# Tamnemng/TAM-GCN

Hardware: AMD Instinct MI355X
Metric: skeleton clips/sec (fwd+CE+bwd+grad all-reduce+SGD step), N-UCLA 20-joint x 64-frame (higher is better)
Workload: dtype f32 (exact fp32-input MFMA v_mfma_f32_16x16x4_f32 in every GEMM, forward and backward: the reference's arithmetic); 1 GPU; N-UCLA joint stream, 256 clips/GPU x (3,64,20,1), models.ctrgcn.Model fwd+CE+bwd+grad-allreduce+SGD step, train-mode BN; global_batch=256, streams=1, parallelism=dp1, launch=hipgraph, model_streams=0, rehearsal=False, allreduce=one flat bucket after backward

## Files before the change

### tam_gcn_amd/csrc/conv.hip

```cpp
#include "common.h"

namespace {

constexpr int BM = 64;
constexpr int BK = 16;
constexpr int BKP = BK + 1;
constexpr int MAXCW = 5;
constexpr int MAXCOLS = 320;

TG_TRACE_DEFINE(tamgcn_trace_read)

struct ConvArgs {
    SrcDev src;
    int N, K, T_in, V;
    const float* w; const float* bias;
    int M, KT, dil, stride, pad;
    long long ws_m, ws_k, ws_t, w_off;
    int up, wmode;
    float* y; int yctot, ycoff, T_out, T_y, ostride;
    const float* add1; const float* add2; const float* bcast; float bcast_scale;
    SrcDev mask; int has_mask;
    const float* aux; const float* aux_center; int auxctot, auxcoff;
    float* stats_part; int stats_ctot, stats_coff, nparts;
    const float* post_coef; int post_ctot, post_act;
// ... 118 lines not shown
    const int V = a.V;
    const int bt = min(a.BT, a.T_out - t0);
    const int ncols = bt * V;
    const int nct = (ncols + 15) >> 4;
    const int cw0 = wave * a.CW;
    const int mt_act = min(4, (min(BM, a.M - m0) + 15) >> 4);
    int c_act = nct - cw0; c_act = c_act < 0 ? 0 : (c_act > a.CW ? a.CW : c_act);

    int boff[MAXCW], tl[MAXCW], vv[MAXCW];
#pragma unroll
    for (int c = 0; c < MAXCW; ++c) {
        int col = (cw0 + c) * 16 + j;
        if (col < ncols) { tl[c] = col / V; vv[c] = col - tl[c] * V; boff[c] = tl[c] * a.sB * V + vv[c]; }
        else { tl[c] = 0; vv[c] = 0; boff[c] = 0; }
    }

    f32x4 acc[4][MAXCW];
#pragma unroll
    for (int mt = 0; mt < 4; ++mt)
#pragma unroll
        for (int c = 0; c < MAXCW; ++c) acc[mt][c] = (f32x4){0.f, 0.f, 0.f, 0.f};

    const int tin0 = t0 * a.stride - a.pad;
    const long long chan_stride = (long long)a.T_in * V;
    const long long src_n = (long long)n * a.src.ctot * chan_stride;

    for (int k0 = 0; k0 < a.K; k0 += BK) {
        __syncthreads();
        const int nA = a.KT * BM * BK;
        for (int e = tid; e < nA; e += NTHREADS) {
            int kk = e & (BK - 1);
            int i = (e >> 4) & (BM - 1);
            int tap = e >> 10;
            int m = m0 + i, k = k0 + kk;
            float wv = 0.f;
            if (m < a.M && k < a.K) wv = a.w[m * a.ws_m + k * a.ws_k + tap * a.ws_t + a.w_off];
            As[(tap * BM + i) * BKP + kk] = wv;
        }
        for (int pos = tid; pos < a.LB; pos += NTHREADS) {
            int slot = pos / V;
            int v = pos - slot * V;
            int th = tin0 + slot * a.lstride;
            bool ok = th >= 0;
            if (a.up > 1) { ok = ok && (th % a.up == 0); th /= a.up; }
            ok = ok && th < a.T_in;
            long long goff = src_n + (long long)th * V + v;
#pragma unroll 4
            for (int kk = 0; kk < BK; ++kk) {
                int k = k0 + kk;
                float xv = 0.f;
                if (ok && k < a.K) {
                    int ch = a.src.coff + k;
                    xv = src_value(a.src, goff + ch * chan_stride, ch);
                }
                Bs[kk * a.pitchB + pos] = xv;
            }
        }
        __syncthreads();
        for (int tap = 0; tap < a.KT; ++tap) {
            const int tapoff = tap * a.dil * V;
#pragma unroll
            for (int k4 = 0; k4 < BK / 4; ++k4) {
                float av[4];
#pragma unroll
                for (int mt = 0; mt < 4; ++mt)
                    av[mt] = As[(tap * BM + mt * 16 + j) * BKP + k4 * 4 + kq];
                const float* brow = Bs + (k4 * 4 + kq) * a.pitchB + tapoff;
#pragma unroll
                for (int c = 0; c < MAXCW; ++c) {
                    if (c < c_act) {
                        float bv = brow[boff[c]];
#pragma unroll
                        for (int mt = 0; mt < 4; ++mt)
                            if (mt < mt_act) acc[mt][c] = mfma16(av[mt], bv, acc[mt][c]);
                    }
                }
            }
        }
    }

    conv_epilogue(a, acc, Ss, n, m0, t0, ncols, cw0, mt_act, c_act, tl, vv, j, kq, wave, tid);
}

template <int NTH, int PR = 0, typename SIDE = PairArgs>
__device__ __forceinline__ void staged_rows(const ConvArgs& a, const float* Tt, int PT, int RP, int r0, int BMT, int m0, int n, int t0,
                                            int ncols, float* Ss, int Vs, int v0, const SIDE* pa = nullptr) {
    const int tid = threadIdx.x, V = a.V;
    const int TPR = NTH / RP;
    const int row = tid / TPR, seg = tid - row * TPR;
    const int m = m0 + r0 + row;
    const bool flat = Vs == V && a.ostride == 1;
    const bool vecok = flat || (Vs & 3) == 0;
    float p1 = 0.f, p2 = 0.f;
    const bool rowok = r0 + row < BMT && m < a.M;
    if (rowok) {
        float bia = a.bias ? a.bias[m] : 0.f;
        float* yp = a.y;
        const float ctr = a.aux ? a.aux_center[a.auxcoff + m] : 0.f;
        const float pc1 = a.post_coef ? a.post_coef[a.ycoff + m] : 1.f, pc0 = a.post_coef ? a.post_coef[2 * a.post_ctot + a.ycoff + m] : 0.f;
        const float plo = a.post_act == 1 ? 0.f : -__builtin_inff();
        long long ybase = ((long long)n * a.yctot + a.ycoff + m) * a.T_y * V;
        if constexpr (PR == 1) {
            if (m >= pa->M0) {
                const int m1 = m - pa->M0;
                bia = pa->bias1 ? pa->bias1[m1] : 0.f; yp = pa->y1;
                ybase = ((long long)n * pa->yctot1 + pa->ycoff1 + m1) * a.T_y * V;
            }
        }
        const long long mbase = a.has_mask ? ((long long)n * a.mask.ctot + a.mask.coff + m) * a.T_y * V : 0;
        const unsigned char* sb = nullptr;
        if constexpr (PR == 2) sb = pa->bits + ((long long)n * pa->ctot + pa->coff + m) * ((a.T_y * V + 3) >> 2);
        const long long abase = a.aux ? ((long long)n * a.auxctot + a.auxcoff + m) * a.T_y * V : 0;
        const float* bc = a.bcast ? a.bcast + ((long long)m * a.N + n) * V : nullptr;
        float mc1 = 1.f, mc2 = 0.f, mc0 = 0.f;
        if (a.has_mask && a.mask.coef) {
            int mch = a.mask.coff + m;
            mc1 = a.mask.coef[mch]; mc0 = a.mask.coef[2 * a.mask.ctot + mch];
            if (a.mask.x2) mc2 = a.mask.coef[a.mask.ctot + mch];
        }
        const int nc4 = (ncols + 3) >> 2;
        unsigned snib = 0;
        if constexpr (PR == 2) {
            const unsigned char* sp = sb + ((t0 * V) >> 2);
#pragma unroll
            for (int k = 0; k < 6; ++k) {
                const int c = seg + k * TPR;
                snib |= (unsigned)sp[c < nc4 ? c : nc4 - 1] << (4 * k);
            }
        }
        int it = 0;
        for (int c4 = seg; c4 < nc4; c4 += TPR, ++it) {
            const int col = c4 << 2;
            const int fr = col / Vs, v = col - fr * Vs;
            if ((vecok || v + 4 <= Vs) && col + 4 <= ncols) {
                const long long off = (long long)(t0 + fr) * a.ostride * V + v0 + v;
                float4 val = *reinterpret_cast<const float4*>(Tt + row * PT + col);
                val.x = fmaf(pc1, val.x + bia, pc0); val.y = fmaf(pc1, val.y + bia, pc0);
                val.z = fmaf(pc1, val.z + bia, pc0); val.w = fmaf(pc1, val.w + bia, pc0);
                if (bc) {
                    float4 b;
                    if ((V & 3) == 0) b = *reinterpret_cast<const float4*>(bc + v0 + v);
                    else { const int j0 = (v0 + v) % V; b = make_float4(bc[j0], bc[(j0 + 1) % V], bc[(j0 + 2) % V], bc[(j0 + 3) % V]); }
                    val.x = fmaf(b.x, a.bcast_scale, val.x); val.y = fmaf(b.y, a.bcast_scale, val.y);
                    val.z = fmaf(b.z, a.bcast_scale, val.z); val.w = fmaf(b.w, a.bcast_scale, val.w);
                }
                if (a.add1) { float4 t = *reinterpret_cast<const float4*>(a.add1 + ybase + off); val.x += t.x; val.y += t.y; val.z += t.z; val.w += t.w; }
                if (a.add2) { float4 t = *reinterpret_cast<const float4*>(a.add2 + ybase + off); val.x += t.x; val.y += t.y; val.z += t.z; val.w += t.w; }
                val.x = fmaxf(val.x, plo); val.y = fmaxf(val.y, plo); val.z = fmaxf(val.z, plo); val.w = fmaxf(val.w, plo);
                if (a.has_mask) {
                    float4 q = *reinterpret_cast<const float4*>(a.mask.x1 + mbase + off);
                    float4 q2 = make_float4(0.f, 0.f, 0.f, 0.f);
                    if (a.mask.x2) q2 = *reinterpret_cast<const float4*>(a.mask.x2 + mbase + off);
                    if (!(fmaf(mc1, q.x, fmaf(mc2, q2.x, mc0)) > 0.f)) val.x = 0.f;
                    if (!(fmaf(mc1, q.y, fmaf(mc2, q2.y, mc0)) > 0.f)) val.y = 0.f;
                    if (!(fmaf(mc1, q.z, fmaf(mc2, q2.z, mc0)) > 0.f)) val.z = 0.f;
                    if (!(fmaf(mc1, q.w, fmaf(mc2, q2.w, mc0)) > 0.f)) val.w = 0.f;
                }
                if constexpr (PR == 2) {
                    const unsigned q = it < 6 ? snib >> (4 * it) : sb[off >> 2];
                    if (!(q & 1u)) val.x = 0.f;
                    if (!(q & 2u)) val.y = 0.f;
                    if (!(q & 4u)) val.z = 0.f;
                    if (!(q & 8u)) val.w = 0.f;
                }
                if (a.stats_part) {
                    float4 x2 = val;
                    if (a.aux) {
                        x2 = *reinterpret_cast<const float4*>(a.aux + abase + off);
                        x2.x -= ctr; x2.y -= ctr; x2.z -= ctr; x2.w -= ctr;
                    }
                    p1 += (val.x + val.y) + (val.z + val.w);
                    p2 = fmaf(val.x, x2.x, fmaf(val.y, x2.y, fmaf(val.z, x2.z, fmaf(val.w, x2.w, p2))));
                }
                *reinterpret_cast<float4*>(yp + ybase + off) = val;
            } else {
                for (int i = 0; i < 4 && col + i < ncols; ++i) {
                    const int ci = col + i, fi = ci / Vs, vi = ci - fi * Vs;
                    const long long off = (long long)(t0 + fi) * a.ostride * V + v0 + vi;
                    float val = fmaf(pc1, Tt[row * PT + ci] + bia, pc0);
                    if (bc) val = fmaf(bc[(v0 + vi) % V], a.bcast_scale, val);
                    if (a.add1) val += a.add1[ybase + off];
                    if (a.add2) val += a.add2[ybase + off];
                    val = fmaxf(val, plo);
                    if (a.has_mask) {
                        const float q = a.mask.x1[mbase + off], q2 = a.mask.x2 ? a.mask.x2[mbase + off] : 0.f;
                        if (!(fmaf(mc1, q, fmaf(mc2, q2, mc0)) > 0.f)) val = 0.f;
                    }
                    if constexpr (PR == 2) {
                        if (!((sb[off >> 2] >> (off & 3)) & 1u)) val = 0.f;
                    }
                    if (a.stats_part) {
                        const float x2 = a.aux ? a.aux[abase + off] - ctr : val;
                        p1 += val;
                        p2 = fmaf(val, x2, p2);
                    }
                    yp[ybase + off] = val;
                }
            }
        }
    }
    if (a.stats_part) {
        for (int o = 1; o < TPR; o <<= 1) { p1 += __shfl_xor(p1, o); p2 += __shfl_xor(p2, o); }
        if (seg == 0 && rowok) { Ss[r0 + row] = p1; Ss[4 * BM + r0 + row] = p2; }
    }
}

template <int BKV, int MT, int CWT>
__global__ __launch_bounds__(NTHREADS) void conv_kernel_vec(const ConvArgs a) {
    extern __shared__ __attribute__((aligned(16))) float smem[];
    constexpr int BKVP = BKV + 2;
    constexpr int BMT = MT * 16;
    constexpr int NPF = (BKV == 32) ? 10 : 8;
    float* As = smem;
    float* Bs = As + ((a.KT * BMT * BKVP + 3) & ~3);
    float* Ss = Bs + BKV * a.pitchB;
    float* cf = Ss + 2 * 4 * BM;

    const int tid = threadIdx.x, lane = tid & 63, wave = tid >> 6;
    const int j = lane & 15, kq = lane >> 4;
    const int tti = blockIdx.x / a.nsl, sl = blockIdx.x - tti * a.nsl;
    const int n = blockIdx.z, m0 = blockIdx.y * BMT, t0 = tti * a.BT;
    const int V = a.V, Vs = a.Vs, Vp = a.Vp, v0 = sl * Vs;
    const int bt = min(a.BT, a.T_out - t0);
    const int ncols = bt * Vs;
    const int cw0 = wave * CWT;

    for (int e = tid; e < a.K; e += NTHREADS) {
        int ch = a.src.coff + e;
        cf[e] = a.src.coef ? a.src.coef[ch] : 1.f;
        cf[a.K + e] = (a.src.coef && a.src.x2) ? a.src.coef[a.src.ctot + ch] : 0.f;
        cf[2 * a.K + e] = a.src.coef ? a.src.coef[2 * a.src.ctot + ch] : 0.f;
    }

    int boff[CWT], tl[CWT], vv[CWT];
#pragma unroll
    for (int c = 0; c < CWT; ++c) {
        int col = (cw0 + c) * 16 + j;
        if (col < ncols) { tl[c] = col / Vs; vv[c] = col - tl[c] * Vs; boff[c] = tl[c] * a.sB * Vp + vv[c]; }
        else { tl[c] = 0; vv[c] = 0; boff[c] = 0; }
    }
    f32x4 acc[MT][CWT];
#pragma unroll
    for (int mt = 0; mt < MT; ++mt)
#pragma unroll
        for (int c = 0; c < CWT; ++c) acc[mt][c] = (f32x4){0.f, 0.f, 0.f, 0.f};

    const int tin0 = t0 * a.stride - a.pad;
    const long long chan_stride = (long long)a.T_in * V;
    const int LB4 = a.LB >> 2;
    const int nvec = BKV * LB4;
    int p_lds[NPF], p_kk[NPF];
    long long p_g[NPF];
    bool p_ok[NPF];
#pragma unroll
    for (int i = 0; i < NPF; ++i) {
        int e = tid + i * NTHREADS;
        int kk = e / LB4, c4 = e - kk * LB4;
        int pos = c4 << 2;
        int slot = pos / Vp, v = pos - slot * Vp;
        int th = tin0 + slot * a.lstride;
        bool ok = e < nvec && th >= 0;
        if (a.up > 1) { ok = ok && (th % a.up == 0); th /= a.up; }
        ok = ok && th < a.T_in;
        p_ok[i] = ok;
        p_kk[i] = e < nvec ? kk : -1;
        p_lds[i] = kk * a.pitchB + pos;
        p_g[i] = (long long)n * a.src.ctot * chan_stride + (long long)(a.src.coff + kk) * chan_stride + (long long)th * V + v0 + v;
    }
    float4 r1[NPF], r2[NPF];
    const bool has2 = a.src.x2 != nullptr;
    constexpr int KTP = BKV == 16 ? 5 : 1;
    constexpr int NAF = (KTP * BMT * BKV + NTHREADS - 1) / NTHREADS;
    const bool apf = a.KT <= KTP;
    float wr[NAF];
    auto prefetch = [&](int k0) {
#pragma unroll
        for (int i = 0; i < NPF; ++i) {
            r1[i] = make_float4(0.f, 0.f, 0.f, 0.f);
            r2[i] = make_float4(0.f, 0.f, 0.f, 0.f);
            if (p_ok[i] && k0 + p_kk[i] < a.K) {
                long long g = p_g[i] + (long long)k0 * chan_stride;
                r1[i] = *reinterpret_cast<const float4*>(a.src.x1 + g);
                if (has2) r2[i] = *reinterpret_cast<const float4*>(a.src.x2 + g);
            }
        }
        if (apf) {
#pragma unroll
            for (int i = 0; i < NAF; ++i) {
// ... 23 lines not shown
        TG_T(tw); TG_ACC(2, tw - tb);
        const int nA = a.KT * BMT * BKV;
        if (apf) {
#pragma unroll
            for (int i = 0; i < NAF; ++i) {
                int e = tid + i * NTHREADS;
                const int tap = e / (BMT * BKV);
                e -= tap * (BMT * BKV);
                int ii, kk;
                if (a.wmode == 0) { kk = e % BKV; ii = e / BKV; } else { ii = e % BMT; kk = e / BMT; }
                if (tap < a.KT) As[(tap * BMT + ii) * BKVP + kk] = wr[i];
            }
        } else if (a.wmode == 0) {
            for (int e = tid; e < nA; e += NTHREADS) {
                int kk = e % BKV;
                int i = (e / BKV) % BMT;
                int tap = e / (BKV * BMT);
                int m = m0 + i, k = k0 + kk;
                float wv = 0.f;
                if (m < a.M && k < a.K) wv = a.w[m * a.ws_m + k * a.ws_k + tap * a.ws_t + a.w_off];
                As[(tap * BMT + i) * BKVP + kk] = wv;
            }
        } else {
            for (int e = tid; e < nA; e += NTHREADS) {
                int i = e % BMT;
                int kk = (e / BMT) % BKV;
                int tap = e / (BKV * BMT);
                int m = m0 + i, k = k0 + kk;
                float wv = 0.f;
                if (m < a.M && k < a.K) wv = a.w[m * a.ws_m + k * a.ws_k + tap * a.ws_t + a.w_off];
                As[(tap * BMT + i) * BKVP + kk] = wv;
            }
        }
#pragma unroll
        for (int i = 0; i < NPF; ++i) {
            if (p_kk[i] >= 0) {
                int k = k0 + p_kk[i];
                float4 o = make_float4(0.f, 0.f, 0.f, 0.f);
                if (p_ok[i] && k < a.K) {
                    float c1 = cf[k], c2 = cf[a.K + k], c0 = cf[2 * a.K + k];
                    o.x = fmaf(c1, r1[i].x, fmaf(c2, r2[i].x, c0)); o.y = fmaf(c1, r1[i].y, fmaf(c2, r2[i].y, c0));
                    o.z = fmaf(c1, r1[i].z, fmaf(c2, r2[i].z, c0)); o.w = fmaf(c1, r1[i].w, fmaf(c2, r2[i].w, c0));
                    if (a.src.act == 1) { o.x = fmaxf(o.x, 0.f); o.y = fmaxf(o.y, 0.f); o.z = fmaxf(o.z, 0.f); o.w = fmaxf(o.w, 0.f); }
                }
                *reinterpret_cast<float4*>(Bs + p_lds[i]) = o;
            }
        }
        TG_T(tc); TG_ACC(3, tc - tw);
        __syncthreads();
        TG_T(td); TG_ACC(4, td - tc);
        if (k0 + BKV < a.K) prefetch(k0 + BKV);
        TG_T(te); TG_ACC(5, te - td);
        for (int tap = 0; tap < a.KT; ++tap) {
            const float* at = arow + tap * BMT * BKVP;
            const float* bt_ = Bs + kq * a.pitchB + tap * a.dil * Vp;
#pragma unroll
            for (int k4 = 0; k4 < BKV / 4; ++k4) {
                float av[MT], bv[CWT];
#pragma unroll
                for (int mt = 0; mt < MT; ++mt) av[mt] = at[mt * 16 * BKVP + k4 * 4];
#pragma unroll
                for (int c = 0; c < CWT; ++c) bv[c] = bt_[k4 * 4 * a.pitchB + boff[c]];
#pragma unroll
                for (int c = 0; c < CWT; ++c)
#pragma unroll
                    for (int mt = 0; mt < MT; ++mt) acc[mt][c] = mfma16(av[mt], bv[c], acc[mt][c]);
            }
        }
        TG_T(tf); TG_ACC(6, tf - te);
    }
    TG_T(tg0);

    __syncthreads();
    float* Tt = smem;
    constexpr int PT = CWT * 64 + 4;
    const int avail = ((a.KT * BMT * BKVP + 3) & ~3) + BKV * a.pitchB;
    int RP = (avail / PT) & ~15;
    if (RP > BMT) RP = BMT;
    if (RP == 48) RP = 32;
    if (a.stats_part) {
        for (int e = tid; e < 2 * 4 * BM; e += NTHREADS) Ss[e] = 0.f;
    }
    for (int r0 = 0; r0 < BMT; r0 += RP) {
        __syncthreads();
#pragma unroll
        for (int mt = 0; mt < MT; ++mt) {
            const int rl = mt * 16 + kq * 4 - r0;
            if (rl >= 0 && rl < RP) {
#pragma unroll
                for (int c = 0; c < CWT; ++c) {
                    const int col = (cw0 + c) * 16 + j;
#pragma unroll
                    for (int r = 0; r < 4; ++r) Tt[(rl + r) * PT + col] = acc[mt][c][r];
                }
            }
        }
        __syncthreads();
        staged_rows<NTHREADS>(a, Tt, PT, RP, r0, BMT, m0, n, t0, ncols, Ss, Vs, v0);
    }
    if (a.stats_part) {
        __syncthreads();
        if (tid < 2 * BMT) {
            int st = tid / BMT, row = tid - st * BMT;
            int m = m0 + row;
            if (m < a.M) {
                int part = n * gridDim.x + blockIdx.x;
                a.stats_part[((long long)st * a.stats_ctot + a.stats_coff + m) * a.nparts + part] = Ss[st * 4 * BM + row];
            }
        }
    }
}



#ifndef TG_KO
#define TG_KO 0
#endif
constexpr int G_NT = 512, G_BMT = 64, G_PA = 80, G_PBMAX = 320, G_NST = 3, G_CWT = 5;

template <int PAIR> struct GldsSide { typedef PairArgs type; };
template <> struct GldsSide<2> { typedef SignArgs type; };
template <int NSRC, int BK, bool PRO, int NW, int PAIR = 0>
__global__ __launch_bounds__(NW * 64, NW == 8 ? 4 : 2) void conv1x1_glds_kernel(const ConvArgs a, int ntt, int nmt, const typename GldsSide<PAIR>::type pa) {
    constexpr int G_NT = NW * 64, G_MT = 16 / NW;
    extern __shared__ __attribute__((aligned(16))) float smem[];
    constexpr int STG = BK * G_PBMAX * NSRC + BK * G_PA;
    constexpr int NAI = BK / NW;
    constexpr int MAXB = (NSRC * (BK / 4) * 5 + NW - 1) / NW;
    float* cf = smem + G_NST * STG;
    float* Ss = cf + (PRO ? 3 * a.K : 0);

    const int tid = threadIdx.x, lane = tid & 63, wave = tid >> 6;
    const int j = lane & 15, kq = lane >> 4, wm = wave >> 2, wn = wave & 3;
    const int V = a.V, K = a.K, LB = a.LB;
    const int rot = ((LB & 31) + 16) & 31;
    int g, mtile;
    {
        const int L = blockIdx.x, ng = a.N * ntt;
        if ((ng & 7) == 0) { const int xcd = L & 7, i = L >> 3; mtile = i % nmt; g = (i / nmt) * 8 + xcd; }
        else { g = L / nmt; mtile = L - g * nmt; }
    }
    const int n = g / ntt, tt = g - n * ntt;
    const int m0 = mtile * G_BMT, t0 = tt * a.BT;
    const int bt = min(a.BT, a.T_out - t0);
    const int ncols = bt * V;
    const long long TV = (long long)a.T_in * V;

    const int NQ = (LB + 63) >> 6;
    const int ls = a.lstride;
    const float rV_ = 1.0f / (float)V;
    const int NI1 = (BK / 4) * NQ;
    int b_rel[MAXB], b_dst[MAXB];
    bool b_ok[MAXB], b_on[MAXB];
    int nissue = 0;
#pragma unroll
    for (int i = 0; i < MAXB; ++i) {
        const int id = wave + i * NW;
        const bool idok = id < NSRC * NI1;
        const int src = idok ? id / NI1 : 0;
        const int rem = id - src * NI1;
        const int grp = rem / NQ, q = rem - grp * NQ;
        const int f = q * 256 + lane * 4;
        const int r = f / LB, off = f - r * LB;
        int col = off + (r & 1) * rot;
        if (col >= LB) col -= LB;
        b_ok[i] = idok && r < 4 && col < ncols;
        const int scol = ls > 1 ? col + tg_rcp_div(col, rV_) * (ls - 1) * V : col;
        b_rel[i] = (int)((grp * 4 + r) * TV) + scol + src * 0x40000000;
        b_dst[i] = src * (BK * G_PBMAX) + grp * 4 * LB + q * 256;
        b_on[i] = __ballot(b_ok[i]) != 0ull;
        nissue += b_on[i] ? 1 : 0;
    }
    const float* xb1 = a.src.x1 + ((long long)n * a.src.ctot + a.src.coff) * TV + (long long)t0 * ls * V;
    const float* xb2 = NSRC == 2 ? a.src.x2 + ((long long)n * a.src.ctot + a.src.coff) * TV + (long long)t0 * ls * V : nullptr;
    constexpr int RPP = 256 / BK;
    constexpr int NAP0 = G_BMT / RPP;
    const bool wm0 = a.wmode == 0;
    bool a_ok; const float* wbase; int a_dst0 = 0;
    if (wm0) {
        const int ml = lane / (BK / 4), q = lane - ml * (BK / 4);
        const int m = wave * RPP + ml;
        const int f = BK == 16 ? (m >> 1) & 3 : (m >> 2) & 1;
        a_ok = wave < NAP0 && m0 + m < a.M;
        const float* wsel = a.w; int mrow = m0 + (a_ok ? m : 0);
        if constexpr (PAIR == 1) {
            if (mrow >= pa.M0) { wsel = pa.w1; mrow -= pa.M0; }
        }
        wbase = wsel + (long long)mrow * a.ws_m + a.w_off + 4 * (q ^ f);
        a_dst0 = wave * 256;
    } else {
        a_ok = m0 + lane < a.M;
        wbase = a.w + (long long)(m0 + (a_ok ? lane : 0)) * a.ws_m + a.w_off;
    }
    const bool a_on = __ballot(a_ok) != 0ull;
    nissue += wm0 ? (a_on ? 1 : 0) : NAI;

    auto issue = [&](int c) {
        float* st = smem + (c % G_NST) * STG;
        const int k0 = c * BK;
        if (TG_KO & 4) {
        } else if (wm0) {
// ... 100 lines not shown
                pf2 v = {fb[cc], fb[cc + 1]};
                if constexpr (NSRC == 2) v = __builtin_elementwise_fma(C1, v, __builtin_elementwise_fma(C2, (pf2){fb2[cc], fb2[cc + 1]}, C0));
                else v = __builtin_elementwise_fma(C1, v, C0);
                bvs[set][cc] = v[0]; bvs[set][cc + 1] = v[1];
            }
            if constexpr (G_CWT & 1) {
                constexpr int cc = G_CWT - 1;
                if constexpr (NSRC == 2) bvs[set][cc] = fmaf(fc[0], fb[cc], fmaf(fc[1], fb2[cc], fc[2]));
                else bvs[set][cc] = fmaf(fc[0], fb[cc], fc[2]);
            }
            if (relu) {
#pragma unroll
                for (int cc = 0; cc < G_CWT; ++cc) asm("v_max_f32 %0, 0, %0" : "+v"(bvs[set][cc]));
            }
        }
    };
    static_assert((G_MT == 2 || G_MT == 4) && G_CWT == 5, "operand lists below");
#define TG_ACC5(mt_) "+v"(acc[mt_][0]), "+v"(acc[mt_][1]), "+v"(acc[mt_][2]), "+v"(acc[mt_][3]), "+v"(acc[mt_][4])
#define TG_V5(x_) "+v"(x_[0]), "+v"(x_[1]), "+v"(x_[2]), "+v"(x_[3]), "+v"(x_[4])
    auto mm = [&](int cur) {
        if constexpr (G_MT == 2) asm volatile("" : "+v"(fa[cur][0]), "+v"(fa[cur][1]), TG_V5(bvs[cur]) :: "memory");
        else asm volatile("" : "+v"(fa[cur][0]), "+v"(fa[cur][1]), "+v"(fa[cur][2]), "+v"(fa[cur][3]), TG_V5(bvs[cur]) :: "memory");
#pragma unroll
        for (int cc = 0; cc < G_CWT; ++cc)
#pragma unroll
            for (int mt = 0; mt < G_MT; ++mt) acc[mt][cc] = mfma16(fa[cur][mt], bvs[cur][cc], acc[mt][cc]);
    };
    auto fin = [&](int nxt) {
        if constexpr (G_MT == 4) asm volatile("" : TG_ACC5(2), TG_ACC5(3) :: "memory");
        if constexpr (NSRC == 2) asm volatile("" : TG_ACC5(0), TG_ACC5(1), TG_V5(fb), TG_V5(fb2) :: "memory");
        else asm volatile("" : TG_ACC5(0), TG_ACC5(1), TG_V5(fb) :: "memory");
        pro(nxt);
        asm volatile("" : TG_V5(bvs[nxt]));
    };
#undef TG_ACC5
#undef TG_V5
    tg_wait_vmcnt<15>((npre - 1) * nissue);
    asm volatile("s_waitcnt lgkmcnt(0)\n\ts_barrier" ::: "memory");
    rd(0, 0, 0, 0);
    pro(0);
    int stg = 0;
    for (int c = 0; c + 1 < nch; ++c) {
        const int k0 = c * BK;
#pragma unroll
        for (int s_ = 0; s_ + 1 < NK; ++s_) {
            rd((s_ & 1) ^ 1, stg, k0, s_ + 1);
            mm(s_ & 1);
            fin((s_ & 1) ^ 1);
        }
        tg_wait_vmcnt<15>(c + 2 < nch ? nissue : 0);
        asm volatile("s_waitcnt lgkmcnt(0)\n\ts_barrier" ::: "memory");
        if (c + 3 < nch) issue(c + 3);
        stg = stg == G_NST - 1 ? 0 : stg + 1;
        rd(NK & 1, stg, k0 + BK, 0);
        mm((NK - 1) & 1);
        fin(NK & 1);
    }
    {
        const int k0 = (nch - 1) * BK;
#pragma unroll
        for (int s_ = 0; s_ < NK; ++s_) {
            if (s_ + 1 < NK) rd((s_ & 1) ^ 1, stg, k0, s_ + 1);
            mm(s_ & 1);
            if (s_ + 1 < NK) fin((s_ & 1) ^ 1);
        }
    }
    TG_T(tg0);

#if TG_KO & 1
    {
        float ssum = 0.f;
        for (int mt = 0; mt < G_MT; ++mt)
            for (int c = 0; c < G_CWT; ++c) ssum += acc[mt][c][0] + acc[mt][c][1] + acc[mt][c][2] + acc[mt][c][3];
        if (ssum == 123.456f) a.y[tid] = ssum;
        return;
    }
#endif
    constexpr int PT = G_CWT * 64 + 4, RP = 32;
    float* Tt = smem;
    if (a.stats_part) {
        for (int e = tid; e < 2 * 4 * BM; e += G_NT) Ss[e] = 0.f;
    }
    for (int r0 = 0; r0 < G_BMT; r0 += RP) {
        __syncthreads();
#pragma unroll
        for (int mt = 0; mt < G_MT; ++mt) {
            const int rl = wm * (G_MT * 16) + mt * 16 - r0;
            if (rl >= 0 && rl < RP) {
#pragma unroll
                for (int c = 0; c < G_CWT; ++c) {
                    const int col = (wn * G_CWT + c) * 16 + j;
#pragma unroll
                    for (int r = 0; r < 4; ++r) Tt[(rl + kq * 4 + r) * PT + col] = acc[mt][c][r];
                }
            }
        }
        __syncthreads();
        staged_rows<G_NT, PAIR>(a, Tt, PT, RP, r0, G_BMT, m0, n, t0, ncols, Ss, V, 0, &pa);
    }
    if (a.stats_part) {
        __syncthreads();
        if (tid < 2 * G_BMT) {
            int stt = tid / G_BMT, row = tid - stt * G_BMT;
            int m = m0 + row;
            if constexpr (PAIR == 1) {
                if (m < a.M && m >= pa.M0) pa.stats1[((long long)stt * pa.sctot1 + pa.scoff1 + m - pa.M0) * a.nparts + g] = Ss[stt * 4 * BM + row];
                else if (m < a.M) a.stats_part[((long long)stt * a.stats_ctot + a.stats_coff + m) * a.nparts + g] = Ss[stt * 4 * BM + row];
            } else {
                if (m < a.M) a.stats_part[((long long)stt * a.stats_ctot + a.stats_coff + m) * a.nparts + g] = Ss[stt * 4 * BM + row];
            }
        }
    }
    TG_T(tg1); TG_ACC(7, tg1 - tg0); TG_ACC(8, tg1 - tt0); TG_ACC(9, 1);
}


constexpr int GS_BK = 32, GS_NST = 2;

template <int TERMS, bool WM0, int MT>
__global__ __launch_bounds__(G_NT) void conv1x1_glds_split_kernel(const ConvArgs a, int ntt, int nmt) {
    constexpr int GS_MT = MT, GS_BMT = 32 * MT, WROWS = 16 * MT;
    extern __shared__ __attribute__((aligned(16))) float smem[];
    constexpr int BK = GS_BK;
    constexpr int STG = BK * G_PBMAX + BK * GS_BMT;
    constexpr int MAXB = ((BK / 4) * 5 + 7) / 8;
    constexpr int NAP = BK * GS_BMT / 256 / 8;
    constexpr int QR = GS_BMT / 4, RPP = 64 / QR;
    float* cf = smem + GS_NST * STG;
    float* Ss = cf + 3 * a.K;
    float* Bc = Ss + 2 * 4 * BM;

    TG_T(tt0);
    const int tid = threadIdx.x, lane = tid & 63, wave = tid >> 6;
    const int j = lane & 15, kq = lane >> 4, wm = wave >> 2, wn = wave & 3;
    const int V = a.V, K = a.K, LB = a.LB;
    const int rot = ((LB & 31) + 16) & 31;
    int g, mtile;
    {
        const int L = blockIdx.x, ng = a.N * ntt;
        if ((ng & 7) == 0) { const int xcd = L & 7, i = L >> 3; mtile = i % nmt; g = (i / nmt) * 8 + xcd; }
        else { g = L / nmt; mtile = L - g * nmt; }
    }
    const int n = g / ntt, tt = g - n * ntt;
    const int m0 = mtile * GS_BMT, t0 = tt * a.BT;
    const int bt = min(a.BT, a.T_out - t0);
    const int ncols = bt * V;
    const long long TV = (long long)a.T_in * V;

    for (int e = tid; e < K; e += G_NT) {
        int ch = a.src.coff + e;
        cf[e] = a.src.coef ? a.src.coef[ch] : 1.f;
        cf[K + e] = (a.src.coef && a.src.x2) ? a.src.coef[a.src.ctot + ch] : 0.f;
        cf[2 * K + e] = a.src.coef ? a.src.coef[2 * a.src.ctot + ch] : 0.f;
    }
    const bool plain = !a.src.coef;
    const int nsrc = a.src.x2 ? 2 : 1;

    const int NQ = (LB + 63) >> 6, NI1 = (BK / 4) * NQ;
    int b_rel[MAXB], b_dst[MAXB];
    bool b_ok[MAXB], b_on[MAXB];
    int nissue = 0;
#pragma unroll
    for (int i = 0; i < MAXB; ++i) {
        const int id = wave + i * 8;
        const bool idok = id < NI1;
        const int grp = (idok ? id : 0) / NQ, q = (idok ? id : 0) - grp * NQ;
        const int f = q * 256 + lane * 4;
        const int r = f / LB, off = f - r * LB;
        int col = off + (r & 1) * rot;
        if (col >= LB) col -= LB;
        b_ok[i] = idok && r < 4 && col < ncols;
        b_rel[i] = (int)((grp * 4 + r) * TV) + col;
        b_dst[i] = grp * 4 * LB + q * 256;
        b_on[i] = __ballot(b_ok[i]) != 0ull;
        nissue += b_on[i] ? 1 : 0;
    }
    const long long xoff = ((long long)n * a.src.ctot + a.src.coff) * TV + (long long)t0 * V;
    const float* xb1 = a.src.x1 + xoff;
    const float* xb2 = a.src.x2 ? a.src.x2 + xoff : nullptr;
    const int nchk = K / BK;
    int a_rel[NAP], a_dst[NAP];
    bool a_ok[NAP];
#pragma unroll
    for (int i = 0; i < NAP; ++i) {
// ... 39 lines not shown
#pragma unroll
    for (int mt = 0; mt < GS_MT; ++mt) {
        const int m = wm * WROWS + mt * 16 + j;
        aoff[mt] = WM0 ? m : (((m >> 2) ^ ((kq & 1) << 2)) << 2) + (m & 3);
    }
    f32x4 acc[GS_MT][G_CWT];
#pragma unroll
    for (int mt = 0; mt < GS_MT; ++mt)
#pragma unroll
        for (int c = 0; c < G_CWT; ++c) acc[mt][c] = (f32x4){0.f, 0.f, 0.f, 0.f};
    float bsum[GS_MT];
#pragma unroll
    for (int mt = 0; mt < GS_MT; ++mt) bsum[mt] = 0.f;

    __syncthreads();
    const int nch = nsrc * nchk;
    issue(0);
    TG_T(tt1); TG_ACC(0, tt1 - tt0);
    for (int c = 0; c < nch; ++c) {
        TG_T(ta);
        asm volatile("s_waitcnt vmcnt(0)" ::: "memory");
        TG_T(tb); TG_ACC(2, tb - ta);
        asm volatile("s_waitcnt lgkmcnt(0)\n\ts_barrier" ::: "memory");
        TG_T(tc); TG_ACC(4, tc - tb);
        if (c + 1 < nch) issue(c + 1);
        TG_T(td); TG_ACC(5, td - tc);
        const float* st = smem + (c % GS_NST) * STG;
        const float* As = st + BK * G_PBMAX;
        const int k0 = (c % nchk) * BK;
        float cs[8], c0[8];
        if (!plain) {
            const float* cc1 = cf + (c < nchk ? 0 : K) + k0 + kq;
#pragma unroll
            for (int e = 0; e < 8; ++e) { cs[e] = cc1[4 * e]; c0[e] = c < nchk ? cf[2 * K + k0 + 4 * e + kq] : 0.f; }
        }
        bf16x8_t ah[GS_MT], al[GS_MT];
#pragma unroll
        for (int mt = 0; mt < GS_MT; ++mt) {
            f32x4 v0, v1;
            if constexpr (WM0) {
                const int m = aoff[mt];
#pragma unroll
                for (int e = 0; e < 4; ++e) { v0[e] = As[m * BK + 4 * (e ^ (m & 7)) + kq]; v1[e] = As[m * BK + 4 * ((e + 4) ^ (m & 7)) + kq]; }
            } else {
#pragma unroll
                for (int e = 0; e < 4; ++e) { v0[e] = As[(4 * e + kq) * GS_BMT + aoff[mt]]; v1[e] = As[(4 * (e + 4) + kq) * GS_BMT + aoff[mt]]; }
            }
            if (!plain) {
#pragma unroll
                for (int e = 0; e < 4; ++e) {
                    bsum[mt] = fmaf(v0[e], c0[e], fmaf(v1[e], c0[e + 4], bsum[mt]));
                    v0[e] *= cs[e]; v1[e] *= cs[e + 4];
                }
            }
            split_bf16x8(v0, v1, ah[mt], al[mt]);
        }
        TG_T(te); TG_ACC(3, te - td);
#pragma unroll
        for (int cc = 0; cc < G_CWT; ++cc) {
            f32x4 v0, v1;
#pragma unroll
            for (int e = 0; e < 4; ++e) { v0[e] = st[(4 * e + kq) * LB + bslot[cc]]; v1[e] = st[(4 * (e + 4) + kq) * LB + bslot[cc]]; }
            bf16x8_t bh, bl;
            split_bf16x8(v0, v1, bh, bl);
#pragma unroll
            for (int mt = 0; mt < GS_MT; ++mt) acc[mt][cc] = mfma_split(ah[mt], al[mt], bh, bl, acc[mt][cc]);
        }
        TG_T(tf); TG_ACC(6, tf - te);
    }
    TG_T(tg0);

    constexpr int PT = G_CWT * 64 + 4, RP = 32;
    float* Tt = smem;
    if (a.stats_part) {
        for (int e = tid; e < 2 * 4 * BM; e += G_NT) Ss[e] = 0.f;
    }
#pragma unroll
    for (int mt = 0; mt < GS_MT; ++mt) {
        float t = bsum[mt];
        t += __shfl_xor(t, 16); t += __shfl_xor(t, 32);
        if (wn == 0 && kq == 0) Bc[wm * WROWS + mt * 16 + j] = t;
    }
    for (int r0 = 0; r0 < GS_BMT; r0 += RP) {
        __syncthreads();
        if (wm * WROWS <= r0 && r0 < wm * WROWS + WROWS) {
            const int mtb = (r0 - wm * WROWS) / 16;
#pragma unroll
            for (int mt2 = 0; mt2 < 2; ++mt2)
#pragma unroll
                for (int c = 0; c < G_CWT; ++c) {
                    const int col = (wn * G_CWT + c) * 16 + j;
#pragma unroll
                    for (int r = 0; r < 4; ++r) {
                        const f32x4 v = (MT == 2 || mtb == 0) ? acc[mt2][c] : acc[(MT == 2 ? 0 : 2) + mt2][c];
                        Tt[(mt2 * 16 + kq * 4 + r) * PT + col] = v[r] + Bc[r0 + mt2 * 16 + kq * 4 + r];
                    }
                }
        }
        __syncthreads();
        staged_rows<G_NT>(a, Tt, PT, RP, r0, GS_BMT, m0, n, t0, ncols, Ss + 0, V, 0);
    }
    if (a.stats_part) {
        __syncthreads();
        if (tid < 2 * GS_BMT) {
            int stt = tid / GS_BMT, row = tid - stt * GS_BMT;
            int m = m0 + row;
            if (m < a.M) a.stats_part[((long long)stt * a.stats_ctot + a.stats_coff + m) * a.nparts + g] = Ss[stt * 4 * BM + row];
        }
    }
    TG_T(tg1); TG_ACC(7, tg1 - tg0); TG_ACC(8, tg1 - tt0); TG_ACC(9, 1);
}

template <int NSRC, int BK>
constexpr size_t glds_lds_bytes(int K, bool pro = true) {
    return sizeof(float) * ((size_t)G_NST * (BK * G_PBMAX * NSRC + BK * G_PA) + (pro ? 3 * (size_t)K : 0) + 2 * 4 * BM);
}

struct ConvPlan { int BT, CW, TIN, lstride, sB, LB, pitchB, ntt, bk, mt, cwt, Vs, Vp, nsl; bool vec, flat; size_t lds; };

static int gcd_i(int a, int b) { while (b) { int t = a % b; a = b; b = t; } return a; }

static int plan_conv(const tamgcn_conv_desc* d, ConvPlan* p) {
    const int V = d->V;
    if (V < 1 || V > MAXCOLS) return -1;
    p->flat = d->KT == 1 && d->stride == 1 && d->up == 1 && d->pad == 0 && d->T_in == d->T_out;
    p->Vs = V; p->nsl = 1;
    if (!p->flat && d->KT > 1 && V > 32 && V % 16 == 0) { p->Vs = 16; p->nsl = V / 16; }
    p->Vp = p->flat ? V : ((p->Vs + 3) & ~3);
    const bool vec_try = d->K <= 1024 && (p->flat || (p->Vp & 3) == 0);
    int BT = MAXCOLS / p->Vs; if (BT < 1) BT = 1;
    if (BT > d->T_out) BT = d->T_out;
    const int q = 4 / gcd_i(V, 4);
    if (p->flat && q > 1 && BT >= q) BT -= BT % q;
    for (;;) {
        p->BT = BT;
        p->lstride = (d->KT == 1) ? d->stride : 1;
        p->sB = (d->KT == 1) ? 1 : d->stride;
        p->TIN = (d->KT == 1) ? BT : (BT - 1) * d->stride + (d->KT - 1) * d->dil + 1;
        p->LB = p->TIN * p->Vp;
        int pitch = p->LB;
        pitch += ((16 - (pitch & 31)) + 32) & 31;
        p->pitchB = pitch;
        p->CW = ceil_div(ceil_div(BT * p->Vs, 16), 4);
        p->vec = false; p->bk = BK;
        bool slots_short = false;
        if (vec_try && (p->LB & 3) == 0) {
            int lb4 = p->LB / 4;
            int bk = (d->KT == 1 && 32 * lb4 <= 10 * NTHREADS) ? 32 : 16;
            if (bk * lb4 <= ((bk == 32) ? 10 : 8) * NTHREADS) { p->vec = true; p->bk = bk; }
            else slots_short = true;
        }
        p->mt = d->M <= 16 ? 1 : d->M <= 32 ? 2 : (d->M % 64 == 0 ? 4 : (d->M % 48 == 0 ? 3 : 4));
        if (d->KT > 1 && p->mt == 4) p->mt = 2;
        p->cwt = p->CW <= 3 ? 3 : 5;
        if (p->vec) {
            size_t avail = (((size_t)d->KT * p->mt * 16 * (p->bk + 2) + 3) & ~(size_t)3) + (size_t)p->bk * pitch;
            if (avail < (size_t)16 * (p->cwt * 64 + 4)) p->vec = false;
        }
        p->lds = p->vec ? sizeof(float) * ((((size_t)d->KT * p->mt * 16 * (p->bk + 2) + 3) & ~(size_t)3) + (size_t)p->bk * pitch +
                                           2 * 4 * BM + 3 * (size_t)d->K)
                        : sizeof(float) * ((size_t)d->KT * BM * (BK + 1) + (size_t)BK * pitch + 2 * 4 * BM);
        if (slots_short && BT > 1) { BT = BT > 4 ? BT - 2 : BT - 1; if (p->flat && q > 1 && BT >= q) BT -= BT % q; continue; }
        if (p->lds <= 64 * 1024 || BT == 1) break;
        BT = (BT + 1) / 2;
        if (p->flat && q > 1 && BT >= q) BT -= BT % q;
    }
    if (!p->vec) { p->Vs = V; p->nsl = 1; if (p->Vp != V) {
        p->Vp = V; p->LB = p->TIN * V; int pitch = p->LB; pitch += ((16 - (pitch & 31)) + 32) & 31; p->pitchB = pitch;
        p->CW = ceil_div(ceil_div(p->BT * V, 16), 4);
        p->lds = sizeof(float) * ((size_t)d->KT * BM * (BK + 1) + (size_t)BK * pitch + 2 * 4 * BM); } }
    if (p->lds > 160 * 1024 || p->CW > MAXCW) return -1;
    p->ntt = ceil_div(d->T_out, p->BT);
    return 0;
}

}


extern "C" int tamgcn_conv_nparts(const tamgcn_conv_desc* d) {
    ConvPlan p;
    if (!d || plan_conv(d, &p)) return -1;
    return d->N * p.ntt * p.nsl;
}
// ... 164 lines not shown
```

Before: 9378 clips/s.

## Batch epilogue side-input loads and hoist per-row constants before LDS barrier

```diff
diff --git a/tam_gcn_amd/csrc/conv.hip b/tam_gcn_amd/csrc/conv.hip
--- a/tam_gcn_amd/csrc/conv.hip
+++ b/tam_gcn_amd/csrc/conv.hip
@@ -224,8 +224,287 @@
     conv_epilogue(a, acc, Ss, n, m0, t0, ncols, cw0, mt_act, c_act, tl, vv, j, kq, wave, tid);
 }
 
+__device__ __forceinline__ int staged_tid() { int t = threadIdx.x; asm volatile("" : "+v"(t)); return t; }
+
+constexpr int SNIB = 5;
+struct StagedConsts {
+    float bia, ctr, pc1, pc0, mc1, mc2, mc0; unsigned snib;
+};
+struct StagedRow {
+    int row, seg; bool rowok;
+    float bia, ctr, pc1, pc0, plo, mc1, mc2, mc0;
+    float* yrow;
+    long long ybase, mbase, abase;
+    const float* bc; unsigned snib;
+    int m, n;
+};
+
+template <int NTH>
+__device__ __forceinline__ int staged_row_m(const ConvArgs& a, int RP, int r0, int BMT, int m0, bool& rowok) {
+    const int row = staged_tid() / (NTH / RP);
+    rowok = r0 + row < BMT && m0 + r0 + row < a.M;
+    return rowok ? m0 + r0 + row : m0;
+}
+
 template <int NTH, int PR = 0, typename SIDE = PairArgs>
-__device__ __forceinline__ void staged_rows(const ConvArgs& a, const float* Tt, int PT, int RP, int r0, int BMT, int m0, int n, int t0,
+__device__ __forceinline__ StagedConsts staged_row_consts(const ConvArgs& a, int RP, int r0, int BMT, int m0, int n, int t0, int ncols,
+                                                          const SIDE* pa = nullptr) {
+    StagedConsts k;
+    const int V = a.V, TPR = NTH / RP;
+    bool rowok;
+    const int m = staged_row_m<NTH>(a, RP, r0, BMT, m0, rowok);
+    k.bia = a.bias ? a.bias[m] : 0.f;
+    if constexpr (PR == 1) {
+        if (m >= pa->M0) k.bia = pa->bias1 ? pa->bias1[m - pa->M0] : 0.f;
+    }
+    k.ctr = a.aux ? a.aux_center[a.auxcoff + m] : 0.f;
+    k.pc1 = a.post_coef ? a.post_coef[a.ycoff + m] : 1.f; k.pc0 = a.post_coef ? a.post_coef[2 * a.post_ctot + a.ycoff + m] : 0.f;
+    k.mc1 = 1.f; k.mc2 = 0.f; k.mc0 = 0.f;
+    if (a.has_mask && a.mask.coef) {
+        int mch = a.mask.coff + m;
+        k.mc1 = a.mask.coef[mch]; k.mc0 = a.mask.coef[2 * a.mask.ctot + mch];
+        if (a.mask.x2) k.mc2 = a.mask.coef[a.mask.ctot + mch];
+    }
+    k.snib = 0;
+    if constexpr (PR == 2) {
+        const int nc4 = (ncols + 3) >> 2, seg = staged_tid() % TPR;
+        const unsigned char* sp = pa->bits + ((long long)n * pa->ctot + pa->coff + m) * ((a.T_y * V + 3) >> 2) + ((t0 * V) >> 2);
+#pragma unroll
+        for (int i = 0; i < SNIB; ++i) {
+            const int c = seg + i * TPR;
+            k.snib |= (unsigned)sp[c < nc4 ? c : nc4 - 1] << (4 * i);
+        }
+    }
+    return k;
+}
+
+template <int NTH, int PR = 0, typename SIDE = PairArgs>
+__device__ __forceinline__ StagedRow staged_row(const ConvArgs& a, const StagedConsts& c, int RP, int r0, int BMT, int m0, int n, const SIDE* pa = nullptr) {
+    StagedRow k;
+    const int tid = staged_tid(), V = a.V, TPR = NTH / RP;
+    k.row = tid / TPR; k.seg = tid - k.row * TPR;
+    const int m = staged_row_m<NTH>(a, RP, r0, BMT, m0, k.rowok);
+    k.bia = c.bia; k.ctr = c.ctr; k.pc1 = c.pc1; k.pc0 = c.pc0; k.mc1 = c.mc1; k.mc2 = c.mc2; k.mc0 = c.mc0; k.snib = c.snib;
+    k.plo = a.post_act == 1 ? 0.f : -__builtin_inff();
+    float* yp = a.y;
+    k.ybase = ((long long)n * a.yctot + a.ycoff + m) * a.T_y * V;
+    if constexpr (PR == 1) {
+        if (m >= pa->M0) { yp = pa->y1; k.ybase = ((long long)n * pa->yctot1 + pa->ycoff1 + m - pa->M0) * a.T_y * V; }
+    }
+    k.yrow = yp + k.ybase;
+    k.mbase = a.has_mask ? ((long long)n * a.mask.ctot + a.mask.coff + m) * a.T_y * V : 0;
+    k.m = m; k.n = n;
+    k.abase = a.aux ? ((long long)n * a.auxctot + a.auxcoff + m) * a.T_y * V : 0;
+    k.bc = a.bcast ? a.bcast + ((long long)m * a.N + n) * V : nullptr;
+    return k;
+}
+
+template <typename SIDE>
+__device__ __forceinline__ const unsigned char* staged_sb(const ConvArgs& a, const StagedRow& k, const SIDE* pa) {
+    if constexpr (std::is_same<SIDE, SignArgs>::value) return pa->bits + ((long long)k.n * pa->ctot + pa->coff + k.m) * ((a.T_y * a.V + 3) >> 2);
+    else return nullptr;
+}
+
+template <int PR, typename SIDE>
+__device__ __forceinline__ void staged_group_cols(const ConvArgs& a, const StagedRow& k, const SIDE* pa, const float* Tr, int col, int ncols, int Vs, int v0,
+                                                  int t0, float& p1, float& p2) {
+    const int V = a.V;
+    for (int i = 0; i < 4 && col + i < ncols; ++i) {
+        const int ci = col + i, fi = ci / Vs, vi = ci - fi * Vs;
+        const long long off = (long long)(t0 + fi) * a.ostride * V + v0 + vi;
+        float val = fmaf(k.pc1, Tr[ci] + k.bia, k.pc0);
+        if (k.bc) val = fmaf(k.bc[(v0 + vi) % V], a.bcast_scale, val);
+        if (a.add1) val += a.add1[k.ybase + off];
+        if (a.add2) val += a.add2[k.ybase + off];
+        val = fmaxf(val, k.plo);
+        if (a.has_mask) {
+            const float q = a.mask.x1[k.mbase + off], q2 = a.mask.x2 ? a.mask.x2[k.mbase + off] : 0.f;
+            if (!(fmaf(k.mc1, q, fmaf(k.mc2, q2, k.mc0)) > 0.f)) val = 0.f;
+        }
+        if constexpr (PR == 2) {
+            if (!((staged_sb(a, k, pa)[off >> 2] >> (off & 3)) & 1u)) val = 0.f;
+        }
+        if (a.stats_part) {
+            const float x2 = a.aux ? a.aux[k.abase + off] - k.ctr : val;
+            p1 += val;
+            p2 = fmaf(val, x2, p2);
+        }
+        k.yrow[off] = val;
+    }
+}
+
+template <int PR, typename SIDE>
+__device__ __forceinline__ void staged_groups_any(const ConvArgs& a, const StagedRow& k, const SIDE* pa, const float* Tr, int TPR, int ncols, int Vs, int v0,
+                                                  int t0, bool vecok, float& p1, float& p2) {
+    const int V = a.V, nc4 = (ncols + 3) >> 2;
+    if (!k.rowok) return;
+    for (int c4 = k.seg; c4 < nc4; c4 += TPR) {
+        const int col = c4 << 2;
+        const int fr = col / Vs, v = col - fr * Vs;
+        if ((vecok || v + 4 <= Vs) && col + 4 <= ncols) {
+            const long long off = (long long)(t0 + fr) * a.ostride * V + v0 + v;
+            float4 val = *reinterpret_cast<const float4*>(Tr + col);
+            val.x = fmaf(k.pc1, val.x + k.bia, k.pc0); val.y = fmaf(k.pc1, val.y + k.bia, k.pc0);
+            val.z = fmaf(k.pc1, val.z + k.bia, k.pc0); val.w = fmaf(k.pc1, val.w + k.bia, k.pc0);
+            if (k.bc) {
+                float4 b;
+                if ((V & 3) == 0) b = *reinterpret_cast<const float4*>(k.bc + v0 + v);
+                else { const int j0 = (v0 + v) % V; b = make_float4(k.bc[j0], k.bc[(j0 + 1) % V], k.bc[(j0 + 2) % V], k.bc[(j0 + 3) % V]); }
+                val.x = fmaf(b.x, a.bcast_scale, val.x); val.y = fmaf(b.y, a.bcast_scale, val.y);
+                val.z = fmaf(b.z, a.bcast_scale, val.z); val.w = fmaf(b.w, a.bcast_scale, val.w);
+            }
+            if (a.add1) { float4 t = *reinterpret_cast<const float4*>(a.add1 + k.ybase + off); val.x += t.x; val.y += t.y; val.z += t.z; val.w += t.w; }
+            if (a.add2) { float4 t = *reinterpret_cast<const float4*>(a.add2 + k.ybase + off); val.x += t.x; val.y += t.y; val.z += t.z; val.w += t.w; }
+            val.x = fmaxf(val.x, k.plo); val.y = fmaxf(val.y, k.plo); val.z = fmaxf(val.z, k.plo); val.w = fmaxf(val.w, k.plo);
+            if (a.has_mask) {
+                float4 q = *reinterpret_cast<const float4*>(a.mask.x1 + k.mbase + off);
+                float4 q2 = make_float4(0.f, 0.f, 0.f, 0.f);
+                if (a.mask.x2) q2 = *reinterpret_cast<const float4*>(a.mask.x2 + k.mbase + off);
+                if (!(fmaf(k.mc1, q.x, fmaf(k.mc2, q2.x, k.mc0)) > 0.f)) val.x = 0.f;
+                if (!(fmaf(k.mc1, q.y, fmaf(k.mc2, q2.y, k.mc0)) > 0.f)) val.y = 0.f;
+                if (!(fmaf(k.mc1, q.z, fmaf(k.mc2, q2.z, k.mc0)) > 0.f)) val.z = 0.f;
+                if (!(fmaf(k.mc1, q.w, fmaf(k.mc2, q2.w, k.mc0)) > 0.f)) val.w = 0.f;
+            }
+            if constexpr (PR == 2) {
+                const unsigned q = staged_sb(a, k, pa)[off >> 2];
+                if (!(q & 1u)) val.x = 0.f;
+                if (!(q & 2u)) val.y = 0.f;
+                if (!(q & 4u)) val.z = 0.f;
+                if (!(q & 8u)) val.w = 0.f;
+            }
+            if (a.stats_part) {
+                float4 x2 = val;
+                if (a.aux) {
+                    x2 = *reinterpret_cast<const float4*>(a.aux + k.abase + off);
+                    x2.x -= k.ctr; x2.y -= k.ctr; x2.z -= k.ctr; x2.w -= k.ctr;
+                }
+                p1 += (val.x + val.y) + (val.z + val.w);
+                p2 = fmaf(val.x, x2.x, fmaf(val.y, x2.y, fmaf(val.z, x2.z, fmaf(val.w, x2.w, p2))));
+            }
+            *reinterpret_cast<float4*>(k.yrow + off) = val;
+        } else {
+            staged_group_cols<PR>(a, k, pa, Tr, col, ncols, Vs, v0, t0, p1, p2);
+        }
+    }
+}
+
+template <int OPS, int NB, int PR, bool BV4 = true, typename SIDE>
+__device__ __forceinline__ void staged_groups(const ConvArgs& a, const StagedRow& k, const SIDE* pa, const float* Tr, int TPR, int ncols, int Vs, int v0, int t0,
+                                              float& p1, float& p2) {
+    constexpr bool hb = OPS & 1, h1 = OPS & 2, h2 = OPS & 4, hm = OPS & 8, hm2 = OPS & 16, hx = OPS & 32;
+    const int V = a.V, nc4 = (ncols + 3) >> 2;
+    const int ngr = (nc4 + TPR - 1) / TPR;
+    const bool st = a.stats_part != nullptr;
+    const float* const pb = k.bc;
+    const float* const q1 = a.add1 + k.ybase;
+    const float* const q2 = a.add2 + k.ybase;
+    const float* const qm = a.mask.x1 + k.mbase;
+    const float* const qm2 = a.mask.x2 + k.mbase;
+    const float* const qx = a.aux + k.abase;
+    for (int it0 = 0; it0 < ngr; it0 += NB) {
+        float4 ob[NB], o1[NB], o2[NB], om[NB], om2[NB], ox[NB];
+        unsigned off[NB];
+        bool vec[NB];
+#pragma unroll
+        for (int i = 0; i < NB; ++i) {
+            const int c4 = k.seg + (it0 + i) * TPR, col = c4 << 2;
+            const int fr = col / Vs, v = col - fr * Vs;
+            vec[i] = k.rowok && col + 4 <= ncols;
+            const int frc = vec[i] ? fr : 0, vc = vec[i] ? v : 0;
+            off[i] = (unsigned)((t0 + frc) * a.ostride * V + v0 + vc);
+            if constexpr (hb) {
+                if constexpr (BV4) ob[i] = *reinterpret_cast<const float4*>(pb + v0 + vc);
+                else { const int j0 = (v0 + vc) % V; ob[i] = make_float4(pb[j0], pb[(j0 + 1) % V], pb[(j0 + 2) % V], pb[(j0 + 3) % V]); }
+            }
+            if constexpr (h1) o1[i] = *reinterpret_cast<const float4*>(q1 + off[i]);
+            if constexpr (h2) o2[i] = *reinterpret_cast<const float4*>(q2 + off[i]);
+            if constexpr (hm) om[i] = *reinterpret_cast<const float4*>(qm + off[i]);
+            if constexpr (hm2) om2[i] = *reinterpret_cast<const float4*>(qm2 + off[i]);
+            if constexpr (hx) ox[i] = *reinterpret_cast<const float4*>(qx + off[i]);
+        }
+#pragma unroll
+        for (int i = 0; i < NB; ++i) {
+            const int col = (k.seg + (it0 + i) * TPR) << 2;
+            if (vec[i]) {
+                float4 val = *reinterpret_cast<const float4*>(Tr + col);
+                val.x = fmaf(k.pc1, val.x + k.bia, k.pc0); val.y = fmaf(k.pc1, val.y + k.bia, k.pc0);
+                val.z = fmaf(k.pc1, val.z + k.bia, k.pc0); val.w = fmaf(k.pc1, val.w + k.bia, k.pc0);
+                if constexpr (hb) {
+                    val.x = fmaf(ob[i].x, a.bcast_scale, val.x); val.y = fmaf(ob[i].y, a.bcast_scale, val.y);
+                    val.z = fmaf(ob[i].z, a.bcast_scale, val.z); val.w = fmaf(ob[i].w, a.bcast_scale, val.w);
+                }
+                if constexpr (h1) { val.x += o1[i].x; val.y += o1[i].y; val.z += o1[i].z; val.w += o1[i].w; }
+                if constexpr (h2) { val.x += o2[i].x; val.y += o2[i].y; val.z += o2[i].z; val.w += o2[i].w; }
+                val.x = fmaxf(val.x, k.plo); val.y = fmaxf(val.y, k.plo); val.z = fmaxf(val.z, k.plo); val.w = fmaxf(val.w, k.plo);
+                if constexpr (hm) {
+                    const float4 q = om[i];
+                    float4 s2 = make_float4(0.f, 0.f, 0.f, 0.f);
+                    if constexpr (hm2) s2 = om2[i];
+                    if (!(fmaf(k.mc1, q.x, fmaf(k.mc2, s2.x, k.mc0)) > 0.f)) val.x = 0.f;
+                    if (!(fmaf(k.mc1, q.y, fmaf(k.mc2, s2.y, k.mc0)) > 0.f)) val.y = 0.f;
+                    if (!(fmaf(k.mc1, q.z, fmaf(k.mc2, s2.z, k.mc0)) > 0.f)) val.z = 0.f;
+                    if (!(fmaf(k.mc1, q.w, fmaf(k.mc2, s2.w, k.mc0)) > 0.f)) val.w = 0.f;
+                }
+                if constexpr (PR == 2) {
+                    const int it = it0 + i;
+                    const unsigned q = it < SNIB ? k.snib >> (4 * it) : staged_sb(a, k, pa)[off[i] >> 2];
+                    if (!(q & 1u)) val.x = 0.f;
+                    if (!(q & 2u)) val.y = 0.f;
+                    if (!(q & 4u)) val.z = 0.f;
+                    if (!(q & 8u)) val.w = 0.f;
+                }
+                if (st) {
+                    float4 x2 = val;
+                    if constexpr (hx) { x2 = ox[i]; x2.x -= k.ctr; x2.y -= k.ctr; x2.z -= k.ctr; x2.w -= k.ctr; }
+                    p1 += (val.x + val.y) + (val.z + val.w);
+                    p2 = fmaf(val.x, x2.x, fmaf(val.y, x2.y, fmaf(val.z, x2.z, fmaf(val.w, x2.w, p2))));
+                }
+                *reinterpret_cast<float4*>(k.yrow + off[i]) = val;
+            }
+        }
+    }
+}
+
+template <int NTH, int NB, int PR = 0, typename SIDE = PairArgs>
+__device__ __forceinline__ void staged_rows(const ConvArgs& a, const StagedConsts& kc, const float* Tt, int PT, int RP, int r0, int BMT, int m0, int n,
+                                            int t0, int ncols, float* Ss, int Vs, int v0, const SIDE* pa = nullptr) {
+    const int V = a.V, TPR = NTH / RP;
+    const StagedRow k = staged_row<NTH, PR>(a, kc, RP, r0, BMT, m0, n, pa);
+    const bool flat = Vs == V && a.ostride == 1;
+    const bool vecok = flat || (Vs & 3) == 0;
+    float p1 = 0.f, p2 = 0.f;
+    const float* Tr = Tt + k.row * PT;
+    const int nc4 = (ncols + 3) >> 2;
+    constexpr bool WHOLE = PR == 2;
+    bool whole_only = true;
+    if (__ballot(k.rowok) == 0ull) {
+        whole_only = false;
+    } else if (!WHOLE && (!vecok || ncols < 4)) {
+        staged_groups_any<PR>(a, k, pa, Tr, TPR, ncols, Vs, v0, t0, vecok, p1, p2);
+        whole_only = false;
+    } else if constexpr (PR == 1) {
+        staged_groups<0, NB, PR>(a, k, pa, Tr, TPR, ncols, Vs, v0, t0, p1, p2);
+    } else {
+        constexpr int N2 = NB < 3 ? NB : 3, N3 = NB < 2 ? NB : 2;
+        const int ops = (a.bcast ? 1 : 0) | (a.add1 ? 2 : 0) | (a.add2 ? 4 : 0) | (a.has_mask ? (a.mask.x2 ? 24 : 8) : 0) | (a.aux && a.stats_part ? 32 : 0);
+        if (PR == 0 && ops == 0) staged_groups<0, NB, 0>(a, k, pa, Tr, TPR, ncols, Vs, v0, t0, p1, p2);
+        else if (ops == 2) staged_groups<2, NB, PR>(a, k, pa, Tr, TPR, ncols, Vs, v0, t0, p1, p2);
+        else if (PR == 0 && ops == 7 && (V & 3) == 0) staged_groups<7, N3, 0, true>(a, k, pa, Tr, TPR, ncols, Vs, v0, t0, p1, p2);
+        else if (PR == 0 && ops == 7) staged_groups<7, N3, 0, false>(a, k, pa, Tr, TPR, ncols, Vs, v0, t0, p1, p2);
+        else if (PR == 0 && ops == 40) staged_groups<40, N2, 0>(a, k, pa, Tr, TPR, ncols, Vs, v0, t0, p1, p2);
+        else if (PR == 0 && ops == 56) staged_groups<56, N3, 0>(a, k, pa, Tr, TPR, ncols, Vs, v0, t0, p1, p2);
+        else { staged_groups_any<PR>(a, k, pa, Tr, TPR, ncols, Vs, v0, t0, vecok, p1, p2); whole_only = false; }
+    }
+    if (!WHOLE && whole_only && (ncols & 3) && k.rowok && (nc4 - 1 - k.seg) % TPR == 0 && nc4 - 1 >= k.seg)
+        staged_group_cols<PR>(a, k, pa, Tr, (nc4 - 1) << 2, ncols, Vs, v0, t0, p1, p2);
+    if (a.stats_part) {
+        for (int o = 1; o < TPR; o <<= 1) { p1 += __shfl_xor(p1, o); p2 += __shfl_xor(p2, o); }
+        if (k.seg == 0 && k.rowok) { Ss[r0 + k.row] = p1; Ss[4 * BM + r0 + k.row] = p2; }
+    }
+}
+#ifdef TAMGCN_EPILOGUE_PER_GROUP
+template <int NTH, int PR = 0, typename SIDE = PairArgs>
+__device__ __forceinline__ void staged_rows_per_group(const ConvArgs& a, const float* Tt, int PT, int RP, int r0, int BMT, int m0, int n, int t0,
                                             int ncols, float* Ss, int Vs, int v0, const SIDE* pa = nullptr) {
     const int tid = threadIdx.x, V = a.V;
     const int TPR = NTH / RP;
@@ -346,6 +625,7 @@
         if (seg == 0 && rowok) { Ss[r0 + row] = p1; Ss[4 * BM + r0 + row] = p2; }
     }
 }
+#endif
 
 template <int BKV, int MT, int CWT>
 __global__ __launch_bounds__(NTHREADS) void conv_kernel_vec(const ConvArgs a) {
@@ -535,6 +815,9 @@
         for (int e = tid; e < 2 * 4 * BM; e += NTHREADS) Ss[e] = 0.f;
     }
     for (int r0 = 0; r0 < BMT; r0 += RP) {
+#ifndef TAMGCN_EPILOGUE_PER_GROUP
+        const StagedConsts rk = staged_row_consts<NTHREADS>(a, RP, r0, BMT, m0, n, t0, ncols);
+#endif
         __syncthreads();
 #pragma unroll
         for (int mt = 0; mt < MT; ++mt) {
@@ -549,7 +832,11 @@
             }
         }
         __syncthreads();
-        staged_rows<NTHREADS>(a, Tt, PT, RP, r0, BMT, m0, n, t0, ncols, Ss, Vs, v0);
+#ifdef TAMGCN_EPILOGUE_PER_GROUP
+        staged_rows_per_group<NTHREADS>(a, Tt, PT, RP, r0, BMT, m0, n, t0, ncols, Ss, Vs, v0);
+#else
+        staged_rows<NTHREADS, 5>(a, rk, Tt, PT, RP, r0, BMT, m0, n, t0, ncols, Ss, Vs, v0);
+#endif
     }
     if (a.stats_part) {
         __syncthreads();
@@ -570,6 +857,11 @@
 #define TG_KO 0
 #endif
 constexpr int G_NT = 512, G_BMT = 64, G_PA = 80, G_PBMAX = 320, G_NST = 3, G_CWT = 5;
+#ifdef TAMGCN_EPILOGUE_PER_GROUP
+#define TG_LDS_BARRIER() __syncthreads()
+#else
+#define TG_LDS_BARRIER() asm volatile("s_waitcnt lgkmcnt(0)\n\ts_barrier" ::: "memory")
+#endif
 
 template <int PAIR> struct GldsSide { typedef PairArgs type; };
 template <> struct GldsSide<2> { typedef SignArgs type; };
@@ -836,7 +1128,10 @@
         for (int e = tid; e < 2 * 4 * BM; e += G_NT) Ss[e] = 0.f;
     }
     for (int r0 = 0; r0 < G_BMT; r0 += RP) {
-        __syncthreads();
+#ifndef TAMGCN_EPILOGUE_PER_GROUP
+        const StagedConsts rk = staged_row_consts<G_NT, PAIR>(a, RP, r0, G_BMT, m0, n, t0, ncols, &pa);
+#endif
+        TG_LDS_BARRIER();
 #pragma unroll
         for (int mt = 0; mt < G_MT; ++mt) {
             const int rl = wm * (G_MT * 16) + mt * 16 - r0;
@@ -849,11 +1144,16 @@
                 }
             }
         }
-        __syncthreads();
-        staged_rows<G_NT, PAIR>(a, Tt, PT, RP, r0, G_BMT, m0, n, t0, ncols, Ss, V, 0, &pa);
+        TG_LDS_BARRIER();
+#ifdef TAMGCN_EPILOGUE_PER_GROUP
+        staged_rows_per_group<G_NT, PAIR>(a, Tt, PT, RP, r0, G_BMT, m0, n, t0, ncols, Ss, V, 0, &pa);
+#else
+        staged_rows<G_NT, 5, PAIR>(a, rk, Tt, PT, RP, r0, G_BMT, m0, n, t0, ncols, Ss, V, 0, &pa);
+#endif
     }
     if (a.stats_part) {
         __syncthreads();
+        const int tid = staged_tid();
         if (tid < 2 * G_BMT) {
             int stt = tid / G_BMT, row = tid - stt * G_BMT;
             int m = m0 + row;
@@ -1059,7 +1359,10 @@
         if (wn == 0 && kq == 0) Bc[wm * WROWS + mt * 16 + j] = t;
     }
     for (int r0 = 0; r0 < GS_BMT; r0 += RP) {
-        __syncthreads();
+#ifndef TAMGCN_EPILOGUE_PER_GROUP
+        const StagedConsts rk = staged_row_consts<G_NT>(a, RP, r0, GS_BMT, m0, n, t0, ncols);
+#endif
+        TG_LDS_BARRIER();
         if (wm * WROWS <= r0 && r0 < wm * WROWS + WROWS) {
             const int mtb = (r0 - wm * WROWS) / 16;
 #pragma unroll
@@ -1074,8 +1377,12 @@
                     }
                 }
         }
-        __syncthreads();
-        staged_rows<G_NT>(a, Tt, PT, RP, r0, GS_BMT, m0, n, t0, ncols, Ss + 0, V, 0);
+        TG_LDS_BARRIER();
+#ifdef TAMGCN_EPILOGUE_PER_GROUP
+        staged_rows_per_group<G_NT>(a, Tt, PT, RP, r0, GS_BMT, m0, n, t0, ncols, Ss + 0, V, 0);
+#else
+        staged_rows<G_NT, 5>(a, rk, Tt, PT, RP, r0, GS_BMT, m0, n, t0, ncols, Ss + 0, V, 0);
+#endif
     }
     if (a.stats_part) {
         __syncthreads();
```

Result: no change. 9382 clips/s (median of 2 runs) (+0.0%).
